# keonlee9420/Transformer-tacotron2

Measured on AMD Instinct MI355X. Metric: mel frames/sec (train step) at 1/2/4/8 GPUs; decode frames/sec b=32, higher is better.
Workload: dtype bf16; 1 GPU; train step (fwd+loss+bwd+Adam; one rank: no gradient exchange), LJSpeech-shape synthetic batch; global_batch=16, per_gpu_batch=16, seq_len=800, text_len=128, n_mels=80, params=52986691, parallelism=dp1, graph=True, optimizer=Adam at the end of each step

## Files before the change

transformer-tacotron2_amd/csrc/gemm.hip:

```cpp
#include "gemm_common.h"

using tt2g::Epilogue;
using tt2g::Operand;

#ifndef TT2_G10_AUTO
#define TT2_G10_AUTO 1
#endif
#ifndef TT2_G11_AUTO
#define TT2_G11_AUTO 1
#endif
#ifndef G11_MAX_K
#define G11_MAX_K 1024
#endif

extern "C" size_t tt2_gemm_workspace_size(const tt2_gemm_args* a) {
  if (a->splits <= 1) return 0;
  return (size_t)a->splits * a->m * (a->n + (a->a_ksum ? 1 : 0)) * sizeof(float);
}

static bool g7_lds_epi(int variant) { return variant != 13; }

#ifndef G8_SPLIT_TO_V7
#define G8_SPLIT_TO_V7 1
#endif
#ifndef G8_AUTO_TILES
#define G8_AUTO_TILES 64
#endif
#ifndef G8_SPLIT_MIN_K
#define G8_SPLIT_MIN_K 4096
#endif
namespace tt2g {
int gemm_plan(const tt2_gemm_args* a) {
  const int var = a->kernel_variant;
  const int64_t a_inner = a->trans_a ? a->m : a->k, b_inner = a->trans_b ? a->n : a->k;
  const bool half_in = a->dtype_in == TT2_BF16 || a->dtype_in == TT2_F16;
  const bool skinny = half_in && a->m <= 64 && !a->trans_a && !a->trans_b && a->k % 8 == 0 &&
                      a->a_conv_t == 0 && (a->splits <= 1 || a->main_only) && (var == 0 || var == 3);
  if (skinny && a->splits > 1 && (a->a_ln_gamma || a->kv_cache || a->pe_table || a->emit_mel ||
                                  a->k % (32 * a->splits) != 0))
    return tt2_set_error(TT2_E_INVALID, "tt2_gemm: skinny split-K slabs need k % (32 splits) == 0, no fusions"), -1;
  if ((a->a_ln_gamma || a->kv_cache) && !skinny)
    return tt2_set_error(TT2_E_INVALID, "tt2_gemm: a_ln / kv fusions need the skinny path (bf16, m <= 64, NT)"), -1;
  if (a->dtype_in == TT2_F16 && !skinny)
    return tt2_set_error(TT2_E_INVALID, "tt2_gemm: f16 operands only on the skinny decode path (m <= 64, NT)"), -1;
  if (a->a_ln_gamma && (a->dtype_in != TT2_BF16 || a->k != 512 || a->lda != a->k || a->m > 32 || !a->a_ln_branch ||
                        !a->a_ln_beta ||
                        !a->a_ln_out))
    return tt2_set_error(TT2_E_INVALID, "tt2_gemm: a_ln needs k == lda == 512, m <= 32, branch, beta and out"), -1;
  if (a->kv_cache && (!a->kv_t || a->dtype_out != a->dtype_in))
    return tt2_set_error(TT2_E_INVALID, "tt2_gemm: kv scatter needs kv_t and an output of the input dtype"), -1;
  if ((a->pe_table || a->emit_mel) && !skinny)
    return tt2_set_error(TT2_E_INVALID, "tt2_gemm: pe / emit epilogues need the skinny path (bf16, m <= 64, NT)"), -1;
  if (a->pe_table && (!a->pe_alpha || !a->pe_t))
    return tt2_set_error(TT2_E_INVALID, "tt2_gemm: pe epilogue needs pe_alpha and pe_t"), -1;
  if (a->emit_mel && (!a->emit_stop || !a->emit_prev || !a->emit_t || !a->emit_done || a->emit_nmels >= a->n ||
                      a->emit_nmels <= 0 || a->emit_tmax <= 0))
    return tt2_set_error(TT2_E_INVALID, "tt2_gemm: emit epilogue needs stop/prev/t/done and n > emit_nmels"), -1;
  if (skinny) return 3;
  const bool v2 = a->dtype_in == TT2_BF16 && var != 1 && a_inner % 8 == 0 && b_inner % 8 == 0;
  if (a->a_ksum && !(v2 && a->trans_a && a->a_conv_t == 0))
    return tt2_set_error(TT2_E_INVALID, "tt2_gemm: a_ksum needs bf16, trans_a, no conv A, the LDS-DMA kernel"), -1;
  if (!v2) return 1;
  auto conv_ok = [](int t, int c) { return t == 0 || (t >= 64 && c >= 64); };
  const bool v7ok = conv_ok(a->a_conv_t, a->a_conv_c) && conv_ok(a->b_conv_t, a->b_conv_c) &&
                    (int64_t)(a->trans_a ? a->k : a->m) * a->lda * 2 < (1LL << 31) &&
                    (int64_t)(a->trans_b ? a->k : a->n) * a->ldb * 2 < (1LL << 31);
  const bool v8ok = !a->trans_a && !a->a_ksum && a->b_conv_t == 0 && a->dtype_out == TT2_BF16 && a->n % 8 == 0 &&
                    !(a->splits > 1 && a->main_only) &&
                    (int64_t)a->m * a->lda * 2 < (1LL << 31) &&
                    (int64_t)(a->trans_b ? a->k : a->n) * a->ldb * 2 < (1LL << 31);
  const int64_t tiles7 = (int64_t)((a->m + 255) / 256) * ((a->n + 127) / 128);
  const bool split_v7 = G8_SPLIT_TO_V7 && a->splits > 1 && v7ok && a->k >= G8_SPLIT_MIN_K;
  if (v8ok && a->m >= 64 && (var == 15 || (var == 0 && tiles7 <= G8_AUTO_TILES && !split_v7))) return 15;
  const bool v10ok = v7ok && !a->trans_a && !a->trans_b && a->a_conv_t == 0 && !a->a_ksum &&
                     a->dtype_out == TT2_BF16 && a->splits <= 1 && a->n % 256 == 0 && a->k % 64 == 0 &&
                     !a->res && !a->gate && a->beta == 0.f && a->act != ACT_TANH &&
                     reinterpret_cast<uintptr_t>(a->c) % 16 == 0 && a->ldc % 8 == 0 &&
                     reinterpret_cast<uintptr_t>(a->bias) % 16 == 0;
  const int64_t cus = tt2_cu_count();
  const int64_t rounds7 = (tiles7 + cus - 1) / cus, rounds10 = ((a->m + 255) / 256 * (a->n / 256) + cus - 1) / cus;
  if (v10ok && (var == 16 || (var == 0 && TT2_G10_AUTO && 17 * rounds10 < 10 * rounds7))) return 16;
  const bool v11ok = v7ok && !a->trans_a && a->a_conv_t == 0 && a->b_conv_t == 0 && !a->a_ksum &&
                     a->dtype_out == TT2_BF16 && a->splits <= 1 && a->n % 128 == 0 && a->k % 64 == 0 &&
                     a->beta == 0.f && a->act != ACT_TANH && !a->col_stats && !a->bn_bwd &&
                     (a->trans_b ? !a->bias && !a->act && !a->drop_thr && !(a->res && a->gate)
                                 : !a->res && !a->gate) &&
                     reinterpret_cast<uintptr_t>(a->c) % 16 == 0 && a->ldc % 8 == 0 &&
                     reinterpret_cast<uintptr_t>(a->bias) % 16 == 0;
  if (v11ok && (var == 17 || (var == 0 && TT2_G11_AUTO && a->k <= G11_MAX_K && !a->trans_b))) return 17;
  if ((var == 13 || var == 14 || var == 0) && v7ok) return 13;
  return 2;
}
}

extern "C" int tt2_gemm_plan(const tt2_gemm_args* a) { return tt2g::gemm_plan(a); }

static bool epi_vec_ok(const tt2_gemm_args* a) {
  auto ok = [](const void* p, int64_t ld, int dt) {
    if (!p) return true;
    const int esz = dt == TT2_BF16 ? 2 : 4;
    return reinterpret_cast<uintptr_t>(p) % 16 == 0 && (ld * esz) % 16 == 0 && (8 * esz) % 16 == 0;
  };
  return a->dtype_out != TT2_F16 && a->res_dtype != TT2_F16 && a->gate_dtype != TT2_F16 &&
         ok(a->c, a->ldc, a->dtype_out) && ok(a->res, a->ldr, a->res_dtype) && ok(a->gate, a->ldg, a->gate_dtype) &&
         (reinterpret_cast<uintptr_t>(a->bias) % 16 == 0);
}

struct Route { int kernel, code, stats_rows; };

static int replan(const tt2_gemm_args* a, int variant) {
  tt2_gemm_args b = *a;
  b.kernel_variant = variant;
  return tt2g::gemm_plan(&b);
}

static Route gemm_route(const tt2_gemm_args* a, bool stats) {
  Route r{tt2g::gemm_plan(a), 0, 0};
  if (r.kernel < 0) return r;
  const bool vec = epi_vec_ok(a);
  if (r.kernel == 15 && !vec) r.kernel = replan(a, 13);
  if (stats) {
    auto al = [](const void* p, int64_t ld) { return reinterpret_cast<uintptr_t>(p) % 16 == 0 && (ld * 2) % 16 == 0; };
    bool ok = a->splits <= 1 && a->dtype_out == TT2_BF16 && al(a->c, a->ldc) && a->n % 8 == 0 &&
              (reinterpret_cast<uintptr_t>(a->col_stats) & 3) == 0;
    if (ok && r.kernel != 15) {
      ok = (r.kernel == 13 || replan(a, 14) == 13) && !a->trans_a && !a->trans_b &&
           g7_lds_epi(a->kernel_variant) && a->n % 128 == 0;
      if (ok) r.kernel = 13;
    }
    r.stats_rows = !ok ? 0 : r.kernel == 15 ? 64 : 256;
    return r;
  }
  if (r.kernel == 16 && (r.code = tt2g::g10_code(a, vec)) < 0) r.kernel = replan(a, 13);
  if (r.kernel == 17 && (r.code = tt2g::g11_code(a, vec)) < 0) r.kernel = replan(a, 13);
  return r;
}

extern "C" int32_t tt2_gemm_stats_rows(const tt2_gemm_args* a) { return gemm_route(a, true).stats_rows; }

int tt2g::gemm_prep(const tt2_gemm_args* a, Operand& A, Operand& B, Epilogue& ep) {
  const int esz = a->dtype_in == TT2_F32 ? 4 : 2;
  const int E = 16 / esz;
  auto misaligned = [&](const void* p, int64_t ld) {
    return (reinterpret_cast<uintptr_t>(p) % 16) != 0 || (ld * esz) % 16 != 0;
  };
  if (!a->a || !a->b || !a->c) return tt2_set_error(TT2_E_INVALID, "tt2_gemm: null operand");
  if (misaligned(a->a, a->lda) || misaligned(a->b, a->ldb))
    return tt2_set_error(TT2_E_INVALID, "tt2_gemm: operands must be 16-B aligned with 16-B multiple leading dims");
  if (a->a_conv_t > 0 && (a->trans_a || a->a_conv_c % E != 0 || a->lda != a->a_conv_c))
    return tt2_set_error(TT2_E_INVALID, "tt2_gemm: conv A needs K-contiguous A, lda == C, C % chunk == 0");
  if (a->b_conv_t > 0 && (!a->trans_b || a->b_conv_c % E != 0 || a->ldb != a->b_conv_c))
    return tt2_set_error(TT2_E_INVALID, "tt2_gemm: conv B needs N-contiguous B, ldb == C, C % chunk == 0");
  if (a->splits > 1 && (!a->workspace || a->ws_bytes < tt2_gemm_workspace_size(a)))
    return tt2_set_error(TT2_E_INVALID, "tt2_gemm: split-K workspace too small");

  A = Operand{a->a, a->lda, 0, 0, a->a_conv_t, a->a_conv_c, a->a_conv_pad};
  B = Operand{a->b, a->ldb, 0, 0, a->b_conv_t, a->b_conv_c, a->b_conv_pad};
  if (!a->trans_a) { A.outer_max = a->m; A.inner_max = a->k; } else { A.outer_max = a->k; A.inner_max = a->m; }
  if (!a->trans_b) { B.outer_max = a->n; B.inner_max = a->k; } else { B.outer_max = a->k; B.inner_max = a->n; }
  if (a->k <= 0) return tt2_set_error(TT2_E_INVALID, "tt2_gemm: k must be > 0");

  ep = Epilogue{};
  ep.c = a->c; ep.ldc = a->ldc; ep.c_dt = a->dtype_out;
  ep.bias = a->bias;
  ep.res = a->res; ep.ldr = a->ldr; ep.res_dt = a->res_dtype;
  ep.gate = a->gate; ep.ldg = a->ldg; ep.gate_dt = a->gate_dtype; ep.gate_scale = a->gate_scale;
  ep.alpha = a->alpha; ep.beta = a->beta; ep.act = a->act;
  ep.drop = drop_of(a);
  if (ep.drop.thr && !ep.drop.seed) return tt2_set_error(TT2_E_INVALID, "tt2_gemm: dropout without seed");
  ep.n_log = a->n;
  ep.ksum = a->a_ksum;
  ep.ksum_beta = a->a_ksum_beta;
  ep.main_only = a->main_only;
  ep.cstats = a->col_stats;
  if (const tt2_bn_args* bn = a->bn_bwd) {
    if (bn->dtype != TT2_DT_BF16 || bn->c != a->n || bn->m != a->m || !bn->y || !bn->mean || !bn->rstd ||
        !bn->gamma || !bn->beta || !bn->workspace || a->col_stats || (bn->drop_thr && !bn->drop_seed))
      return tt2_set_error(TT2_E_INVALID, "tt2_gemm: bn_bwd needs a bf16 BatchNorm of this GEMM's m x n, its "
                                          "y / mean / rstd / gamma / beta, a chunk-sums workspace, no col_stats");
    ep.bnb.y = reinterpret_cast<const bf16*>(bn->y);
    ep.bnb.mean = bn->mean; ep.bnb.rstd = bn->rstd; ep.bnb.gamma = bn->gamma; ep.bnb.beta = bn->beta;
    ep.bnb.part = reinterpret_cast<float*>(bn->workspace);
    ep.bnb.drop = drop_of(bn);
    ep.bnb.act = bn->act;
  }
  ep.vec = epi_vec_ok(a);
  return TT2_OK;
}

extern "C" int tt2_gemm(const tt2_gemm_args* a, hipStream_t stream) {
  ProbeDisarm disarm;
  if (a->m <= 0 || a->n <= 0) return TT2_OK;
  Operand A, B;
  Epilogue ep;
  if (const int rc = tt2g::gemm_prep(a, A, B, ep); rc != TT2_OK) return rc;
  float* ws = reinterpret_cast<float*>(a->workspace);
  const int sp = a->splits > 1 ? a->splits : 1;
  const bool stats = ep.cstats || ep.bnb.part;
  const Route r = gemm_route(a, stats);
  if (r.kernel < 0) return TT2_E_INVALID;
  if (stats) {
    if (!r.stats_rows)
      return tt2_set_error(TT2_E_INVALID, "tt2_gemm: col_stats / bn_bwd need the v8 path or v7's LDS-image path "
                                          "(bf16 C, 16-B aligned rows, no split-K; v7: NT and n % 128 == 0)");
    const int rp = r.stats_rows;
    if (a->bn_bwd && a->bn_bwd->ws_bytes < (size_t)((a->m + rp - 1) / rp) * 2 * a->n * sizeof(float))
      return tt2_set_error(TT2_E_INVALID, "tt2_gemm: bn_bwd workspace smaller than its chunk sums");
  }
  const bool a_kc = !a->trans_a, b_kc = !a->trans_b;
  const int m = a->m, n = a->n, k = a->k;
  switch (r.kernel) {
    case 3:
      return tt2_check_launch(tt2g::launch_skinny(a, ep, stream), "tt2_gemm(skinny)");
    case 16:
      return tt2_check_launch(tt2g::launch10(A, B, ep, m, n, k, r.code, stream), "tt2_gemm(v10)");
    case 17:
      return tt2_check_launch(tt2g::launch11(A, B, ep, m, n, k, b_kc, r.code, stream), "tt2_gemm(v11)");
    case 15:
      return tt2_check_launch(tt2g::launch8(b_kc, A, B, ep, m, n, k, stream), "tt2_gemm(v8)");
    case 13:
      return tt2_check_launch(tt2g::launch7(a_kc, b_kc, A, B, ep, m, n, k, sp, ws, stream,
                                            g7_lds_epi(a->kernel_variant)), "tt2_gemm(v7)");
    case 2:
      return tt2_check_launch(tt2g::launch2(a_kc, b_kc, A, B, ep, m, n, k, sp, ws, stream), "tt2_gemm");
    default:
      return tt2_check_launch(tt2g::launch1(a->dtype_in == TT2_BF16, a_kc, b_kc, A, B, ep, m, n, k, sp, ws, stream),
                              "tt2_gemm");
  }
}
```

transformer-tacotron2_amd/csrc/gemm_common.h:

```cpp
#pragma once
#include <hip/hip_ext.h>

#include <algorithm>
#include <cstdlib>

#include "tt2_common.h"
#include "tt2_capi.h"
#include "tt2_internal.h"

#ifdef TT2_PHASE
#define TT2_SPAN_W 32
#else
#define TT2_SPAN_W 2
#endif

namespace tt2g {

struct Operand {
  const void* p;
  int64_t ld;
  int outer_max, inner_max;
  int conv_t, conv_c, conv_pad;
};

struct Epilogue {
  void* c; int64_t ldc; int c_dt;
  const float* bias;
  const void* res; int64_t ldr; int res_dt;
  const void* gate; int64_t ldg; int gate_dt; float gate_scale;
  float alpha, beta;
  int act;
  DropDesc drop;
  int n_log;
  int vec;
  float* ksum; float ksum_beta;
  int main_only;
  float* cstats;
  struct {
    const bf16* y; const float* mean; const float* rstd; const float* gamma; const float* beta;
    float* part;
    DropDesc drop;
    int act;
  } bnb;
};

int probe_take(hipEvent_t& e0, hipEvent_t& e1, unsigned long long*& span, int groups);
void probe_chunk(int slot, int wgs);
void probe_disarm();

hipError_t launch1(bool bf16_in, bool a_kc, bool b_kc, const Operand& A, const Operand& B, const Epilogue& E, int M,
                   int N, int K, int splits, float* ws, hipStream_t s);
hipError_t launch2(bool a_kc, bool b_kc, const Operand& A, const Operand& B, const Epilogue& E, int M, int N, int K,
                   int splits, float* ws, hipStream_t s);
void launch_splitk_reduce(const float* ws, int splits, const Epilogue& E, int M, int N, hipStream_t s);
int splitk_blocks(int M, int N, const Epilogue& E);
hipError_t launch_skinny(const tt2_gemm_args* a, const Epilogue& E, hipStream_t s);
hipError_t launch7(bool a_kc, bool b_kc, const Operand& A, const Operand& B, const Epilogue& E, int M, int N, int K,
                   int splits, float* ws, hipStream_t s, bool lds_epi);
hipError_t launch8(bool b_kc, const Operand& A, const Operand& B, const Epilogue& E, int M, int N, int K,
                   hipStream_t s);
int g10_code(const tt2_gemm_args* a, bool vec);
hipError_t launch10(const Operand& A, const Operand& B, const Epilogue& E, int M, int N, int K, int code,
                    hipStream_t s);
int g11_code(const tt2_gemm_args* a, bool vec);
hipError_t launch11(const Operand& A, const Operand& B, const Epilogue& E, int M, int N, int K, bool b_kc, int code,
                    hipStream_t s);

int gemm_prep(const tt2_gemm_args* a, Operand& A, Operand& B, Epilogue& ep);
int gemm_plan(const tt2_gemm_args* a);

}

namespace {

struct OpDesc : tt2g::Operand {};
struct EpiParams : tt2g::Epilogue {};

constexpr int NT = 256;
constexpr int BM = 128, BN = 128;

TT2_DEV void span_begin(unsigned long long* span, int* done) {
  if (span && threadIdx.x == 0) {
    *done = 0;
    asm volatile("s_waitcnt lgkmcnt(0)" ::: "memory");
    span[TT2_SPAN_W * blockIdx.x] = wall_clock64();
#ifdef TT2_PHASE
    span[TT2_SPAN_W * blockIdx.x + 2] = __builtin_amdgcn_s_memtime();
#endif
  }
}
TT2_DEV void span_end(unsigned long long* span, int* done, int waves) {
  if (span) {
    asm volatile("s_waitcnt vmcnt(0)" ::: "memory");
    if ((threadIdx.x & 63) == 0 && atomicAdd(done, 1) == waves - 1) {
#ifdef TT2_PHASE
      span[TT2_SPAN_W * blockIdx.x + 31] = __builtin_amdgcn_s_memtime();
#endif
      span[TT2_SPAN_W * blockIdx.x + 1] = wall_clock64();
    }
  }
}

struct ProbeScope {
  hipEvent_t e0 = nullptr, e1 = nullptr;
  unsigned long long* span = nullptr;
  int slot = -1;
  ProbeScope(hipStream_t s, int groups) {
    if ((slot = tt2g::probe_take(e0, e1, span, groups)) < 0) return;
    hipStreamCaptureStatus cs = hipStreamCaptureStatusNone;
    if (hipStreamIsCapturing(s, &cs) == hipSuccess && cs == hipStreamCaptureStatusActive) e0 = e1 = nullptr;
    (void)hipGetLastError();
  }
  bool ext() const { return e0 != nullptr; }
  void chunk(int wgs) const { if (slot >= 0) tt2g::probe_chunk(slot, wgs); }
};

struct ProbeDisarm {
  ~ProbeDisarm() { tt2g::probe_disarm(); }
};

TT2_DEV float ld_any(const void* p, int64_t i, int dt) {
  if (dt == TT2_F16) return (float)reinterpret_cast<const f16*>(p)[i];
  return dt == TT2_BF16 ? (float)reinterpret_cast<const bf16*>(p)[i] : reinterpret_cast<const float*>(p)[i];
}
TT2_DEV void st_any(void* p, int64_t i, int dt, float v) {
  if (dt == TT2_F16) reinterpret_cast<f16*>(p)[i] = (f16)v;
  else if (dt == TT2_BF16) reinterpret_cast<bf16*>(p)[i] = (bf16)v;
  else reinterpret_cast<float*>(p)[i] = v;
}

TT2_DEV float epi_value(const EpiParams& e, uint32_t seed, int m, int n, float v) {
  v *= e.alpha;
  if (e.bias) v += e.bias[n];
  if (e.res) v += ld_any(e.res, (int64_t)m * e.ldr + n, e.res_dt);
  if (e.act == ACT_RELU) v = fmaxf(v, 0.f);
  else if (e.act == ACT_TANH) v = tanhf(v);
  if (e.gate) v = ld_any(e.gate, (int64_t)m * e.ldg + n, e.gate_dt) != 0.f ? v * e.gate_scale : 0.f;
  if (e.drop.thr) v = drop_apply(e.drop, seed, (uint32_t)((int64_t)m * e.n_log + n), v);
  if (e.beta != 0.f) v += e.beta * ld_any(e.c, (int64_t)m * e.ldc + n, e.c_dt);
  return v;
}

__device__ __attribute__((aligned(64))) uint4 g_zero_page[64];

typedef __attribute__((address_space(1))) void gvoid_t;
typedef __attribute__((address_space(3))) void lvoid_t;

TT2_DEV int mc_swz(int k) { return ((k & 3) << 1) ^ (((k >> 3) & 1) << 3); }

TT2_DEV const void* chunk_src(const OpDesc& d, int outer, int inner) {
  bool ok = (outer < d.outer_max) & (inner < d.inner_max);
  int64_t off = (int64_t)outer * d.ld + inner;
  if (d.conv_t > 0) {
    const int ts = outer % d.conv_t + inner / d.conv_c - d.conv_pad;
    ok = ok & (ts >= 0) & (ts < d.conv_t);
    off -= (int64_t)d.conv_pad * d.conv_c;
  }
  const void* p = reinterpret_cast<const bf16*>(d.p) + off;
  return ok ? p : (const void*)g_zero_page;
}

template <bool KC>
TT2_DEV void frag2(Frag8<bf16>& f, const char* tile, int r0, int kk, int lane) {
  if (KC) {
    const int row = r0 + (lane & 15);
    const int h = 4 * kk + (lane >> 4);
    f.v = *reinterpret_cast<const bf16x8*>(tile + row * 128 + ((h ^ (row & 7)) << 4));
  } else {
    const int g = lane >> 4, q = (lane >> 2) & 3, p = lane & 3;
    const int c = (r0 + 4 * p) >> 3;
    typedef __attribute__((address_space(3))) short4v lds_s4;
    const int k_lo = 32 * kk + 8 * g + q;
    const int k_hi = k_lo + 4;
    const char* a0 = tile + k_lo * 256 + ((c ^ mc_swz(k_lo)) << 4) + ((p & 1) << 3);
    const char* a1 = tile + k_hi * 256 + ((c ^ mc_swz(k_hi)) << 4) + ((p & 1) << 3);
    short4v lo = __builtin_amdgcn_ds_read_tr16_b64_v4i16((lds_s4*)(a0));
    short4v hi = __builtin_amdgcn_ds_read_tr16_b64_v4i16((lds_s4*)(a1));
    union { short s[8]; bf16x8 v; } u;
    u.s[0] = lo[0]; u.s[1] = lo[1]; u.s[2] = lo[2]; u.s[3] = lo[3];
    u.s[4] = hi[0]; u.s[5] = hi[1]; u.s[6] = hi[2]; u.s[7] = hi[3];
    f.v = u.v;
  }
}

TT2_DEV void ld8_any(const void* p, int64_t off, int dt, float (&o)[8]) {
  if (dt == TT2_BF16) {
    const bf16x8 x = *reinterpret_cast<const bf16x8*>(reinterpret_cast<const bf16*>(p) + off);
#pragma unroll
    for (int j = 0; j < 8; ++j) o[j] = (float)x[j];
  } else {
    const float* q = reinterpret_cast<const float*>(p) + off;
    const f32x4 a = *reinterpret_cast<const f32x4*>(q), b = *reinterpret_cast<const f32x4*>(q + 4);
#pragma unroll
    for (int j = 0; j < 4; ++j) { o[j] = a[j]; o[4 + j] = b[j]; }
  }
}

TT2_DEV void unpack_lds8(const void* p, float (&t)[8]) {
  const bf16x8 x = *reinterpret_cast<const bf16x8*>(p);
#pragma unroll
  for (int j = 0; j < 8; ++j) t[j] = (float)x[j];
}
TT2_DEV void epi_calc8(const EpiParams& E, uint32_t seed, int m, int n0, const float (&v)[8], bool pre_b,
                       float (&o)[8], const void* res_l = nullptr, const void* gate_l = nullptr) {
  const int64_t off = (int64_t)m * E.ldc + n0;
  float t[8];
#pragma unroll
  for (int j = 0; j < 8; ++j) o[j] = pre_b ? v[j] : v[j] * E.alpha;
  if (E.bias && !pre_b) {
    const f32x4 a = *reinterpret_cast<const f32x4*>(E.bias + n0), b = *reinterpret_cast<const f32x4*>(E.bias + n0 + 4);
#pragma unroll
    for (int j = 0; j < 4; ++j) { o[j] += a[j]; o[4 + j] += b[j]; }
  }
  if (E.res) {
    if (res_l) unpack_lds8(res_l, t);
    else ld8_any(E.res, (int64_t)m * E.ldr + n0, E.res_dt, t);
#pragma unroll
    for (int j = 0; j < 8; ++j) o[j] += t[j];
  }
// ... 124 lines not shown
```

transformer-tacotron2_amd/csrc/gemm_v7_impl.h:

```cpp
#pragma once
#include "gemm_v7.h"

namespace {

#ifndef G7_REG
#define G7_REG 0
#endif

template <int NI>
TT2_DEV void g7_put(const u32x4 (&r)[NI], char* lds, int lane, int lw) {
#pragma unroll
  for (int i = 0; i < NI; ++i) *reinterpret_cast<u32x4*>(lds + (lw * NI + i) * 1024 + lane * 16) = r[i];
}

constexpr int G7_MAXP = 8;
struct G7Fin {
  const float* part;
  float* dst[3];
  float gb;
  int nb, C;
};
struct G7Group {
  G7Prob p[G7_MAXP];
  int np, items;
  int ibase;
  G7Fin fin;
  int fin_only;
};
constexpr int G7_FIN_WAVES = 4;

template <int SM>
TT2_DEV void g7_store_c(const G7Prob& P, char* smem, int m0, int n0, int nkt) {
  bf16* C = reinterpret_cast<bf16*>(P.E.c);
  constexpr bool st = SM == 1, sb = SM == 2;
  const int c = threadIdx.x & 15;
  float k[8], s1[8], s2[8];
  if (st) bf16x8_unpack(*reinterpret_cast<const u32x4*>(smem + g7_img_row(nkt, 0) + (c << 4)), k);
#pragma unroll
  for (int j = 0; j < 8; ++j) s1[j] = s2[j] = 0.f;
  constexpr int NR = (256 * 16 + G7_NT - 1) / G7_NT;
  constexpr int YB = NR / 2;
  u32x4 yv[YB];
  float mu[8], rs[8], ga[8], be[8];
  uint32_t seed = 0;
  auto load_y = [&](int i0) {
#pragma unroll
    for (int i = 0; i < YB; ++i) {
      const int r = (threadIdx.x >> 4) + (G7_NT / 16) * (i0 + i), m = min(m0 + r, P.M - 1);
      yv[i] = r < 256 ? *reinterpret_cast<const u32x4*>(P.E.bnb.y + (int64_t)m * P.N + n0 + 8 * c)
                      : u32x4{0, 0, 0, 0};
    }
  };
  if constexpr (sb) {
    const int n = n0 + 8 * c;
    load_y(0);
#pragma unroll
    for (int j = 0; j < 8; ++j) {
      mu[j] = P.E.bnb.mean[n + j]; rs[j] = P.E.bnb.rstd[n + j];
      ga[j] = P.E.bnb.gamma[n + j]; be[j] = P.E.bnb.beta[n + j];
    }
    seed = P.E.bnb.drop.thr ? *P.E.bnb.drop.seed : 0u;
  }
#pragma unroll
  for (int i = 0; i < NR; ++i) {
    if constexpr (sb) {
      if (i == YB) load_y(YB);
    }
    const int id = threadIdx.x + G7_NT * i;
    if (id >= 256 * 16) break;
    const int r = id >> 4, m = m0 + r, n = n0 + 8 * c;
    if (m < P.M && n < P.N) {
      const u32x4 v = *reinterpret_cast<const u32x4*>(smem + g7_img_row(nkt, r) + ((c ^ (r & 15)) << 4));
      u32x4* dst = reinterpret_cast<u32x4*>(C + (int64_t)m * P.E.ldc + n);
      __builtin_nontemporal_store(v, dst);
      if constexpr (st) {
        float f[8];
        bf16x8_unpack(v, f);
#pragma unroll
        for (int j = 0; j < 8; ++j) {
          const float d = f[j] - k[j];
          s1[j] += d;
          s2[j] += d * d;
        }
      }
      if constexpr (sb) {
        float d[8], yf[8];
        bf16x8_unpack(v, d);
        bf16x8_unpack(yv[i % YB], yf);
        const DropDesc& dd = P.E.bnb.drop;
        const uint32_t bits = dd.thr ? drop_bits8(seed, dd.site, (uint32_t)((int64_t)m * P.N + n), dd.thr) : 0xFFu;
        const float sc = dd.thr ? dd.scale : 1.f;
#pragma unroll
        for (int j = 0; j < 8; ++j) {
          const float keep = (bits >> j) & 1u ? sc : 0.f;
          const float xh = (yf[j] - mu[j]) * rs[j];
          const float z = act_f(P.E.bnb.act, xh * ga[j] + be[j]);
          const float dp = d[j] * keep * act_grad_from_out(P.E.bnb.act, z);
          s1[j] += dp;
          s2[j] += dp * xh;
        }
      }
    }
  }
  if constexpr (!st && !sb) return;
  else {
#pragma unroll
  for (int j = 0; j < 8; ++j) {
    s1[j] += __shfl_xor(s1[j], 16);
    s2[j] += __shfl_xor(s2[j], 16);
    s1[j] += __shfl_xor(s1[j], 32);
    s2[j] += __shfl_xor(s2[j], 32);
  }
  float* red = reinterpret_cast<float*>(smem + ((nkt + 2) % 3) * G7_STAGE);
  const int lane = threadIdx.x & 63, wave = threadIdx.x >> 6;
  if (lane < 16) {
#pragma unroll
    for (int j = 0; j < 8; ++j) {
      red[(wave * 128 + 8 * c + j) * 2 + 0] = s1[j];
      red[(wave * 128 + 8 * c + j) * 2 + 1] = s2[j];
    }
  }
  __syncthreads();
  const int t = threadIdx.x;
  if (t < 128 && n0 + t < P.N) {
    float S1 = 0.f, S2 = 0.f;
    for (int w = 0; w < G7_NT / 64; ++w) {
      S1 += red[(w * 128 + t) * 2 + 0];
      S2 += red[(w * 128 + t) * 2 + 1];
    }
    const float kt = __uint_as_float((uint32_t)*reinterpret_cast<const uint16_t*>(smem + g7_img_row(nkt, 0) +
                                                                                  2 * t) << 16);
    if constexpr (st) {
      const float nr = (float)min(256, P.M - m0);
      float* out = P.E.cstats + (int64_t)(m0 / 256) * 2 * P.N + n0 + t;
      out[0] = kt + S1 / nr;
      out[P.N] = fmaxf(S2 - S1 * S1 / nr, 0.f);
    } else {
      float* out = P.E.bnb.part + (int64_t)(m0 / 256) * 2 * P.N + n0 + t;
      out[0] = S1;
      out[P.N] = S2;
    }
  }
  }
}

template <bool BIAS, bool RELU, bool DROP, int PX>
TT2_DEV void g7_epi_fast(const EpiParams& E, const f32x4 (&acc)[4][4], const f32x4 (&pbias)[2][2], char* smem,
                         int nkt, int m0, int n0, int wm, int wn, int lane, uint64_t dbits) {
  const int q = lane >> 4;
#pragma unroll
  for (int i = 0; i < 4; ++i) {
    const int r = wm * 64 + 16 * i + (lane & 15), m = m0 + r;
#pragma unroll
    for (int pr = 0; pr < 2; ++pr) {
      float v[8];
#pragma unroll
      for (int rr = 0; rr < 4; ++rr) {
// ... 330 lines not shown
__global__ __launch_bounds__(G7_NT, 1) void gemm7_kernel(G7Prob P) {
  __shared__ __attribute__((aligned(1024))) char smem[G7_SMEM];
  __shared__ int span_done;
  G7_RT(0)
  span_begin(P.span, &span_done);
  const int u = xcd_item(blockIdx.x, P.items);
  g7_item<AK, BKC, SM>(P, u % (P.items / P.splits), u / (P.items / P.splits), smem, P.span);
  span_end(P.span, &span_done, G7_NT / 64);
  G7_RT(1)
}

template <bool AK, bool BKC>
__global__ __launch_bounds__(G7_NT, 1) void gemm7g_kernel(G7Group G) {
  __shared__ __attribute__((aligned(1024))) char smem[G7_SMEM];
  __shared__ int span_done;
  span_begin(G.p[0].span, &span_done);
  const int u = xcd_item(G.ibase + blockIdx.x, G.items);
  int p = 0;
#pragma unroll
  for (int i = 1; i < G7_MAXP; ++i)
    if (i < G.np && u >= G.p[i].item0) p = i;
  const G7Prob& P = G.p[p];
  const int local = u - P.item0, nt = P.items / P.splits;
  g7_item<AK, BKC>(P, local % nt, local / nt, smem, G.p[0].span);
  span_end(G.p[0].span, &span_done, G7_NT / 64);
}

__global__ void gemm_splitk_reduce(const float* ws, int splits, EpiParams E, int M, int N) {
  splitk_reduce_body(ws, splits, E, M, N, blockIdx.x, gridDim.x);
}

__global__ void gemm_splitk_reduce_g(G7Group G) {
  if (G.fin_only || (int)blockIdx.y == G.np) {
    const G7Fin& f = G.fin;
    const int o = blockIdx.x * G7_FIN_WAVES + (threadIdx.x >> 6), lane = threadIdx.x & 63;
    if (o >= 3 * f.C) return;
    const int which = o / f.C, c = o - which * f.C;
    float* dst = f.dst[which];
    if (!dst) return;
    const float* src = f.part + (int64_t)which * f.C + c;
    const int64_t rs = 3 * (int64_t)f.C;
    float acc[4] = {0.f, 0.f, 0.f, 0.f};
    int r = lane;
    for (; r + 192 < f.nb; r += 256) {
#pragma unroll
      for (int u = 0; u < 4; ++u) acc[u] += src[(r + 64 * u) * rs];
    }
    for (; r < f.nb; r += 64) acc[0] += src[r * rs];
    const float v = wave_sum((acc[0] + acc[1]) + (acc[2] + acc[3]));
    if (lane == 0) dst[c] = f.gb != 0.f ? f.gb * dst[c] + v : v;
    return;
  }
  const G7Prob& P = G.p[blockIdx.y];
  if (P.splits > 1) splitk_reduce_body(P.ws, P.splits, P.E, P.M, P.N, blockIdx.x, gridDim.x);
}

G7Prob g7_prob(const OpDesc& A, const OpDesc& B, const EpiParams& E, int M, int N, int K, int splits,
                            float* ws) {
  G7Prob P{A, B, E, M, N, K, K, 1, (N + 127) / 128, 0, 0, ws, 0, 0, -1, nullptr};
  if (splits > 1) {
    P.k_split = ((K + splits - 1) / splits + 63) / 64 * 64;
    P.splits = (K + P.k_split - 1) / P.k_split;
  }
  P.items = ((M + 255) / 256) * P.ntn * P.splits;
  return P;
}

int g7_fast_code(const G7Prob& P, bool fwd) {
  const EpiParams& E = P.E;
  if (!P.lds_epi || E.beta != 0.f || E.act == ACT_TANH) return -1;
  if (P.pre_x) {
    const bool alone = !E.bias && E.act == ACT_NONE && !E.drop.thr && (P.pre_x == 1 ? !E.gate : !E.res);
    return alone ? 7 + P.pre_x : -1;
  }
  if (E.res || E.gate) return -1;
  if (E.bias && !fwd) return -1;
  return (E.bias ? 1 : 0) | (E.act == ACT_RELU ? 2 : 0) | (E.drop.thr ? 4 : 0);
}

template <bool AK, bool BKC>
hipError_t launch7_t(const OpDesc& A, const OpDesc& B, const EpiParams& E, int M, int N, int K, int splits, float* ws,
                   hipStream_t s, bool lds_epi) {
  G7Prob P = g7_prob(A, B, E, M, N, K, splits, ws);
  P.lds_epi = lds_epi && P.splits == 1 && E.c_dt == TT2_BF16 && E.vec && (N % 8) == 0;
  P.pre_x = !P.lds_epi ? 0 : (E.res && E.res_dt == TT2_BF16) ? 1 : (E.gate && E.gate_dt == TT2_BF16) ? 2 : 0;
  P.epi_fast = g7_fast_code(P, AK && BKC);
  ProbeScope ps(s, P.items);
  P.span = ps.span;
  const int sm = E.cstats ? 1 : E.bnb.part ? 2 : 0;
  auto go = [&](auto kern) {
    if (ps.ext()) hipExtLaunchKernelGGL(kern, dim3(P.items), dim3(G7_NT), 0, s, ps.e0, ps.e1, 0, P);
    else hipLaunchKernelGGL(kern, dim3(P.items), dim3(G7_NT), 0, s, P);
  };
  if constexpr (AK && BKC) {
    if (sm == 1) go(gemm7_kernel<AK, BKC, 1>);
    else if (sm == 2) go(gemm7_kernel<AK, BKC, 2>);
    else go(gemm7_kernel<AK, BKC, 0>);
  } else {
    go(gemm7_kernel<AK, BKC, 0>);
  }
  if (P.splits > 1 && !E.main_only)
    tt2g::launch_splitk_reduce(ws, P.splits, E, M, N, s);
  return hipGetLastError();
}

}

namespace tt2g {

void launch_splitk_reduce(const float* ws, int splits, const Epilogue& E, int M, int N, hipStream_t s) {
  hipLaunchKernelGGL(gemm_splitk_reduce, dim3(splitk_blocks(M, N, E)), dim3(256), 0, s, ws, splits, EpiParams{E}, M, N);
}

int splitk_blocks(int M, int N, const Epilogue& E) {
  const int64_t per = ((N & 7) == 0 && E.vec) ? 8 : ((N & 3) == 0 ? 4 : 1);
  const int64_t items = std::max<int64_t>(((int64_t)M * N + per - 1) / per, M);
  const int64_t nb = (items + 255) / 256;
  return (int)(nb < 4096 ? nb : 4096);
}

hipError_t launch7(bool a_kc, bool b_kc, const Operand& A_, const Operand& B_, const Epilogue& E_, int M, int N, int K,
                   int splits, float* ws, hipStream_t s, bool lds_epi) {
  const OpDesc A{A_}, B{B_};
  const EpiParams E{E_};
  if (a_kc && b_kc) return launch7_t<true, true>(A, B, E, M, N, K, splits, ws, s, lds_epi);
  if (a_kc && !b_kc) return launch7_t<true, false>(A, B, E, M, N, K, splits, ws, s, lds_epi);
  if (!a_kc && b_kc) return launch7_t<false, true>(A, B, E, M, N, K, splits, ws, s, lds_epi);
  return launch7_t<false, false>(A, B, E, M, N, K, splits, ws, s, lds_epi);
}

}

extern "C" int tt2_gemm_grouped_fin(const tt2_gemm_args* probs, int n, const tt2_ln_args* fin,
                                    hipStream_t stream) {
  return tt2_gemm_grouped_ex(probs, n, fin, 0, stream);
}

extern "C" int tt2_gemm_grouped_ex(const tt2_gemm_args* probs, int n, const tt2_ln_args* fin, int max_groups,
                                   hipStream_t stream) {
  ProbeDisarm disarm;
  if (n <= 0 && !fin) return TT2_OK;
  if ((n > 0 && !probs) || n > G7_MAXP) return tt2_set_error(TT2_E_INVALID, "tt2_gemm_grouped: 1..8 problems");
  G7Group G{};
  if (fin && fin->m > 0) {
    if (!fin->defer_finalize || !fin->workspace || fin->c <= 0)
      return tt2_set_error(TT2_E_INVALID, "tt2_gemm_grouped_fin: fin must be a deferred LayerNorm backward");
    G.fin.part = reinterpret_cast<const float*>(fin->workspace);
    G.fin.dst[0] = fin->dgamma; G.fin.dst[1] = fin->dbeta; G.fin.dst[2] = fin->dbias;
    G.fin.gb = fin->grad_beta;
    G.fin.C = fin->c;
    G.fin.nb = (int)(tt2_layernorm_bwd_workspace_size(fin) / (3 * sizeof(float) * fin->c));
  }
  int reduce_blocks = 0, ta = -1, tb = -1, main_only = 1;
  for (int i = 0; i < n; ++i) {
    const tt2_gemm_args* a = probs + i;
    if (a->m <= 0 || a->n <= 0) continue;
    OpDesc A, B;
    EpiParams ep;
    if (const int rc = tt2g::gemm_prep(a, A, B, ep); rc != TT2_OK) return rc;
    if (tt2g::gemm_plan(a) != 13)
      return tt2_set_error(TT2_E_INVALID, "tt2_gemm_grouped: every problem must take the v7 kernel (bf16, "
                                          "8-aligned inner dims, conv T, C >= 64, no decode fusions)");
    if (a->col_stats || a->bn_bwd) return tt2_set_error(TT2_E_INVALID, "tt2_gemm_grouped: no col_stats / bn_bwd");
    if (ta < 0) { ta = a->trans_a; tb = a->trans_b; }
    if (a->trans_a != ta || a->trans_b != tb)
      return tt2_set_error(TT2_E_INVALID, "tt2_gemm_grouped: problems must share trans_a / trans_b");
    G7Prob P = g7_prob(A, B, ep, a->m, a->n, a->k, a->splits > 1 ? a->splits : 1,
                       reinterpret_cast<float*>(a->workspace));
    P.item0 = G.items;
    G.items += P.items;
    G.p[G.np++] = P;
    main_only &= a->main_only;
    if (P.splits > 1) {
      reduce_blocks = std::max(reduce_blocks, tt2g::splitk_blocks(a->m, a->n, ep));
    }
  }
  const int fin_blocks = G.fin.nb ? (3 * G.fin.C + G7_FIN_WAVES - 1) / G7_FIN_WAVES : 0;
  if (G.np == 0) {
    G.fin_only = 1;
    if (fin_blocks) hipLaunchKernelGGL(gemm_splitk_reduce_g, dim3(fin_blocks, 1), dim3(256), 0, stream, G);
    return tt2_check_launch(hipGetLastError(), "tt2_gemm_grouped");
  }
  const int grid = max_groups > 0 ? std::min(G.items, std::max(8, max_groups / 8 * 8)) : G.items;
  ProbeScope ps(stream, G.items);
  ps.chunk(grid);
  for (G.ibase = 0; G.ibase < G.items; G.ibase += grid) {
    const dim3 g(std::min(grid, G.items - G.ibase));
    G.p[0].span = ps.span ? ps.span + (size_t)TT2_SPAN_W * G.ibase : nullptr;
    hipEvent_t ev0 = G.ibase == 0 ? ps.e0 : nullptr, ev1 = G.ibase + grid >= G.items ? ps.e1 : nullptr;
#define TT2_G7G(A_, B_)                                                                                    \
  if (ps.ext())                                                                                          \
    hipExtLaunchKernelGGL((gemm7g_kernel<A_, B_>), g, dim3(G7_NT), 0, stream, ev0, ev1, 0, G);            \
  else                                                                                                   \
    hipLaunchKernelGGL((gemm7g_kernel<A_, B_>), g, dim3(G7_NT), 0, stream, G);
    if (!ta && !tb) { TT2_G7G(true, true) }
    else if (!ta && tb) { TT2_G7G(true, false) }
    else if (ta && !tb) { TT2_G7G(false, true) }
    else { TT2_G7G(false, false) }
#undef TT2_G7G
  }
  G.ibase = 0;
  G.p[0].span = nullptr;
  if (main_only) reduce_blocks = 0;
  G.fin_only = reduce_blocks == 0 && fin_blocks > 0;
  if (G.fin_only)
    hipLaunchKernelGGL(gemm_splitk_reduce_g, dim3(fin_blocks, 1), dim3(256), 0, stream, G);
  else if (reduce_blocks > 0)
    hipLaunchKernelGGL(gemm_splitk_reduce_g, dim3(std::max(reduce_blocks, fin_blocks), G.np + (fin_blocks ? 1 : 0)),
                       dim3(256), 0, stream, G);
  return tt2_check_launch(hipGetLastError(), "tt2_gemm_grouped");
}

extern "C" int tt2_gemm_grouped(const tt2_gemm_args* probs, int n, hipStream_t stream) {
  return tt2_gemm_grouped_fin(probs, n, nullptr, stream);
}
```

Baseline: 1.975 million frames/s.

## Add warp-specialized 256x256 TN GEMM kernel for f32-output weight gradients

Adds a new v12 GEMM kernel with 256x256 tiles, 12 waves per block (8 compute, 4 producer waves issuing global-to-LDS loads into a 5-slot ring) and transposed LDS reads, for bf16 TN problems with f32 C. Grouped GEMM calls now route eligible problems (m,n multiples of 256, no split-K, plain epilogue) to it by default, and run the remaining problems on v7 afterwards. The aim is more data reuse per tile and loads that overlap compute on the large weight-gradient GEMMs. In exchange it adds a second launch per grouped call and uses one block per CU with large LDS, which can leave fewer tiles than CUs for some shapes.

Result: no change. 1.991 million frames/s (median of 6 runs) (+0.8%).

```diff
diff --git a/transformer-tacotron2_amd/csrc/gemm.hip b/transformer-tacotron2_amd/csrc/gemm.hip
--- a/transformer-tacotron2_amd/csrc/gemm.hip
+++ b/transformer-tacotron2_amd/csrc/gemm.hip
@@ -65,6 +65,11 @@
   const bool v7ok = conv_ok(a->a_conv_t, a->a_conv_c) && conv_ok(a->b_conv_t, a->b_conv_c) &&
                     (int64_t)(a->trans_a ? a->k : a->m) * a->lda * 2 < (1LL << 31) &&
                     (int64_t)(a->trans_b ? a->k : a->n) * a->ldb * 2 < (1LL << 31);
+  if (var == 18) {
+    if (v7ok && g12_shape_ok(a)) return 18;
+    return tt2_set_error(TT2_E_INVALID, "tt2_gemm: variant 18 needs a v7-eligible TN request with f32 C, m and n "
+                                        "multiples of 256, plain operands, no split-K"), -1;
+  }
   const bool v8ok = !a->trans_a && !a->a_ksum && a->b_conv_t == 0 && a->dtype_out == TT2_BF16 && a->n % 8 == 0 &&
                     !(a->splits > 1 && a->main_only) &&
                     (int64_t)a->m * a->lda * 2 < (1LL << 31) &&
@@ -212,6 +217,11 @@
   switch (r.kernel) {
     case 3:
       return tt2_check_launch(tt2g::launch_skinny(a, ep, stream), "tt2_gemm(skinny)");
+    case 18: {
+      const tt2g::GroupedProb gp{A, B, ep, m, n, k};
+      ProbeScope ps(stream, tt2g::g12_items(&gp, 1));
+      return tt2_check_launch(tt2g::launch12g(&gp, 1, 0, stream, ps.span, ps.e0, ps.e1), "tt2_gemm(v12)");
+    }
     case 16:
       return tt2_check_launch(tt2g::launch10(A, B, ep, m, n, k, r.code, stream), "tt2_gemm(v10)");
     case 17:
diff --git a/transformer-tacotron2_amd/csrc/gemm_common.h b/transformer-tacotron2_amd/csrc/gemm_common.h
--- a/transformer-tacotron2_amd/csrc/gemm_common.h
+++ b/transformer-tacotron2_amd/csrc/gemm_common.h
@@ -65,6 +65,11 @@
 int g11_code(const tt2_gemm_args* a, bool vec);
 hipError_t launch11(const Operand& A, const Operand& B, const Epilogue& E, int M, int N, int K, bool b_kc, int code,
                     hipStream_t s);
+struct GroupedProb { Operand A, B; Epilogue E; int M, N, K; };
+bool g12_shape_ok(const tt2_gemm_args* a);
+int g12_items(const GroupedProb* pr, int np);
+hipError_t launch12g(const GroupedProb* pr, int np, int max_groups, hipStream_t s, unsigned long long* span,
+                     hipEvent_t e0, hipEvent_t e1);
 
 int gemm_prep(const tt2_gemm_args* a, Operand& A, Operand& B, Epilogue& ep);
 int gemm_plan(const tt2_gemm_args* a);
diff --git a/transformer-tacotron2_amd/csrc/gemm_v12.hip b/transformer-tacotron2_amd/csrc/gemm_v12.hip
--- /dev/null
+++ b/transformer-tacotron2_amd/csrc/gemm_v12.hip
@@ -0,0 +1,267 @@
+#include "gemm_v7.h"
+
+namespace {
+
+constexpr int G12_NT = 768;
+constexpr int G12_SLOT = 256 * 128;
+constexpr int G12_SLOTS = 5;
+constexpr int G12_SMEM = G12_SLOTS * G12_SLOT;
+constexpr int G12_MAXP = 8;
+
+struct G12Prob {
+  OpDesc A, B;
+  EpiParams E;
+  int M, N, K, ntn, item0;
+};
+struct G12Group {
+  G12Prob p[G12_MAXP];
+  int np, items;
+  int ibase;
+  unsigned long long* span;
+};
+
+TT2_DEV uint32_t g12_lane_off(int lane) {
+  const int g = lane >> 4, q = (lane >> 2) & 3, p = lane & 3, k = 8 * g + q;
+  return (uint32_t)(k * 256 + (((p >> 1) ^ mc_swz(k)) << 4) + ((p & 1) << 3));
+}
+typedef __attribute__((address_space(3))) char lchar_t;
+TT2_DEV void g12_frag(Frag8<bf16>& fr, const lchar_t* smem, uint32_t off, int fx, int kk) {
+  typedef __attribute__((address_space(3))) short4v lds_s4;
+  const lchar_t* a0 = smem + (off ^ (uint32_t)fx) + 8192 * kk;
+  short4v lo = __builtin_amdgcn_ds_read_tr16_b64_v4i16((lds_s4*)(a0));
+  short4v hi = __builtin_amdgcn_ds_read_tr16_b64_v4i16((lds_s4*)(a0 + 1024));
+  union { short s[8]; bf16x8 v; } u;
+  u.s[0] = lo[0]; u.s[1] = lo[1]; u.s[2] = lo[2]; u.s[3] = lo[3];
+  u.s[4] = hi[0]; u.s[5] = hi[1]; u.s[6] = hi[2]; u.s[7] = hi[3];
+  fr.v = u.v;
+}
+
+typedef uint32_t g12_u32x2 __attribute__((ext_vector_type(2)));
+template <int OFF>
+TT2_DEV g12_u32x2 g12_tr_asm(uint32_t addr) {
+  g12_u32x2 r;
+  asm volatile("ds_read_b64_tr_b16 %0, %1 offset:%2" : "=v"(r) : "v"(addr), "n"(OFF));
+  return r;
+}
+
+TT2_DEV void g12_wait(int n) {
+  if (n >= 24) asm volatile("s_waitcnt vmcnt(24)" ::: "memory");
+  else if (n >= 16) asm volatile("s_waitcnt vmcnt(16)" ::: "memory");
+  else if (n >= 8) asm volatile("s_waitcnt vmcnt(8)" ::: "memory");
+  else asm volatile("s_waitcnt vmcnt(0)" ::: "memory");
+}
+
+__global__ __launch_bounds__(G12_NT, 1) void gemm12g_kernel(G12Group G) {
+  __shared__ __attribute__((aligned(1024))) char smem[G12_SMEM];
+  const int tid = threadIdx.x, lane = tid & 63, wave = __builtin_amdgcn_readfirstlane(tid >> 6);
+  unsigned long long* span = G.span;
+  if (span && tid == 0) span[TT2_SPAN_W * blockIdx.x] = wall_clock64();
+#ifdef TT2_PHASE
+  unsigned long long* srec = span ? span + TT2_SPAN_W * blockIdx.x : nullptr;
+  if (srec && tid == 0) srec[2] = __builtin_amdgcn_s_memtime();
+#endif
+  const int u = xcd_item(G.ibase + blockIdx.x, G.items);
+  int p = 0;
+#pragma unroll
+  for (int i = 1; i < G12_MAXP; ++i)
+    if (i < G.np && u >= G.p[i].item0) p = i;
+  const G12Prob& P = G.p[p];
+  const OpDesc& A = P.A;
+  const OpDesc& B = P.B;
+  const EpiParams& E = P.E;
+  const int tile = u - P.item0, ntn = P.ntn, K = P.K;
+  const int m0 = (tile / ntn) * 256, n0 = (tile % ntn) * 256;
+  const int nkt = (K + 63) / 64, nit = 2 * nkt;
+  if (wave >= 8) {
+    const int lw = wave - 8;
+    const bool tail = (K & 63) != 0;
+    G7Lane<8> la, lb;
+    g7_lane_init<false>(la, A, m0, 0, lane, lw);
+    g7_lane_init<false>(lb, B, n0, 0, lane, lw);
+    auto issue = [&](int it) {
+      char* dst = smem + (it % G12_SLOTS) * G12_SLOT;
+      const int t = it >> 1;
+      const bool tl = tail && t == nkt - 1;
+      if (it & 1) g7_issue<false>(B, lb, dst, 64 * t, K, lane, lw, tl, false);
+      else g7_issue<false>(A, la, dst, 64 * t, K, lane, lw, tl, false);
+    };
+    const bool do_ks = E.ksum && (tile % ntn) == 0;
+    f32x4 ksa[4];
+#pragma unroll
+    for (int ii = 0; ii < 4; ++ii) ksa[ii] = f32x4{0.f, 0.f, 0.f, 0.f};
+    Frag8<bf16> fones;
+#pragma unroll
+    for (int e = 0; e < 8; ++e) fones.v[e] = (bf16)1.f;
+    const uint32_t lk0 = (uint32_t)(uintptr_t)(const lchar_t*)smem +
+                         ((g12_lane_off(lane) + (lw >> 1) * 16384) ^ (uint32_t)((lw & 1) << 7));
+    const int pre = min(G12_SLOTS, nit);
+    for (int it = 0; it < pre; ++it) issue(it);
+    g12_wait(8 * (pre - 2));
+    __builtin_amdgcn_s_barrier();
+    for (int t = 0; t < nkt; ++t) {
+      if (t >= 1) {
+        if (2 * t + 3 < nit) issue(2 * t + 3);
+        if (2 * t + 4 < nit) issue(2 * t + 4);
+      }
+      if (do_ks) {
+        const uint32_t oa = ((2 * t) % G12_SLOTS) * G12_SLOT + lk0;
+        g12_u32x2 r[4][4];
+#pragma unroll
+        for (int ii = 0; ii < 4; ++ii) {
+          const uint32_t a = oa ^ (uint32_t)(ii << 5);
+          r[ii][0] = g12_tr_asm<0>(a);
+          r[ii][1] = g12_tr_asm<1024>(a);
+          r[ii][2] = g12_tr_asm<8192>(a);
+          r[ii][3] = g12_tr_asm<9216>(a);
+        }
+        asm volatile("s_waitcnt lgkmcnt(0)" ::: "memory");
+        __builtin_amdgcn_sched_barrier(0);
+#pragma unroll
+        for (int kk = 0; kk < 2; ++kk)
+#pragma unroll
+          for (int ii = 0; ii < 4; ++ii) {
+            union { g12_u32x2 h[2]; bf16x8 v; } u;
+            u.h[0] = r[ii][2 * kk];
+            u.h[1] = r[ii][2 * kk + 1];
+            Frag8<bf16> fa;
+            fa.v = u.v;
+            mma16(fones, fa, ksa[ii]);
+          }
+      }
+      if (t + 1 < nkt) {
+        const int last = min(nit - 1, max(G12_SLOTS - 1, 2 * t + 4));
+        g12_wait(8 * (last - (2 * t + 3)));
+      }
+      __builtin_amdgcn_s_barrier();
+    }
+    if (do_ks) {
+#pragma unroll
+      for (int ii = 0; ii < 4; ++ii) {
+        const float ks = ksa[ii][0];
+        const int m = m0 + 16 * (4 * lw + ii) + lane;
+        if (lane < 16) E.ksum[m] = E.ksum_beta != 0.f ? E.ksum_beta * E.ksum[m] + ks : ks;
+      }
+    }
+  } else {
+    const int wm = wave >> 2, wn = wave & 3, q = lane >> 4;
+    f32x4 acc[8][4];
+#pragma unroll
+    for (int i = 0; i < 8; ++i)
+#pragma unroll
+      for (int j = 0; j < 4; ++j) acc[i][j] = f32x4{0.f, 0.f, 0.f, 0.f};
+#if G7_PRIO
+    if (wave >= 4) __builtin_amdgcn_s_setprio(1);
+#endif
+    const lchar_t* sl = (const lchar_t*)smem;
+    const uint32_t la0 = g12_lane_off(lane) + wm * 16384;
+    const uint32_t lb0 = (g12_lane_off(lane) ^ (uint32_t)((wn & 1) << 7)) + (wn >> 1) * 16384;
+    __builtin_amdgcn_s_barrier();
+    for (int t = 0; t < nkt; ++t) {
+      G7_STAMP(t, 0)
+      uint32_t oa = ((2 * t) % G12_SLOTS) * G12_SLOT + la0, ob = ((2 * t + 1) % G12_SLOTS) * G12_SLOT + lb0;
+      asm volatile("" : "+v"(oa), "+v"(ob));
+      Frag8<bf16> fb[4], fa[2];
+#pragma unroll
+      for (int j = 0; j < 4; ++j) g12_frag(fb[j], sl, ob, j << 5, 0);
+      g12_frag(fa[0], sl, oa, 0, 0);
+#pragma unroll
+      for (int b = 0; b < 16; ++b) {
+        const int i = b & 7;
+        if (b + 1 < 16) g12_frag(fa[(b + 1) & 1], sl, oa, ((b + 1) & 7) << 5, (b + 1) >> 3);
+#pragma unroll
+        for (int j = 0; j < 4; ++j) {
+          mma16(fb[j], fa[b & 1], acc[i][j]);
+          if (b == 7) g12_frag(fb[j], sl, ob, j << 5, 1);
+        }
+        __builtin_amdgcn_sched_barrier(0);
+      }
+      G7_STAMP(t, 1)
+      asm volatile("s_waitcnt lgkmcnt(0)" ::: "memory");
+      __builtin_amdgcn_s_barrier();
+    }
+    G7_STAMP(nkt, 0)
+    float* C = reinterpret_cast<float*>(E.c);
+    const float alpha = E.alpha, beta = E.beta;
+#pragma unroll
+    for (int i = 0; i < 8; ++i) {
+      const int m = m0 + wm * 128 + 16 * i + (lane & 15);
+#pragma unroll
+      for (int pr = 0; pr < 2; ++pr) {
+        float v[8];
+#pragma unroll
+        for (int r = 0; r < 4; ++r) {
+          const auto sw = __builtin_amdgcn_permlane16_swap(__float_as_uint(acc[i][2 * pr][r]),
+                                                           __float_as_uint(acc[i][2 * pr + 1][r]), false, false);
+          v[r] = __uint_as_float(sw[0]);
+          v[4 + r] = __uint_as_float(sw[1]);
+        }
+        const int n = n0 + wn * 64 + 16 * (2 * pr + (q & 1)) + 8 * (q >> 1);
+        float* c = C + (int64_t)m * E.ldc + n;
+        float o[8];
+#pragma unroll
+        for (int j = 0; j < 8; ++j) o[j] = v[j] * alpha;
+        if (beta != 0.f) {
+          const f32x4 t0 = *reinterpret_cast<const f32x4*>(c), t1 = *reinterpret_cast<const f32x4*>(c + 4);
+#pragma unroll
+          for (int j = 0; j < 4; ++j) { o[j] += beta * t0[j]; o[4 + j] += beta * t1[j]; }
+        }
+        *reinterpret_cast<f32x4*>(c) = f32x4{o[0], o[1], o[2], o[3]};
+        *reinterpret_cast<f32x4*>(c + 4) = f32x4{o[4], o[5], o[6], o[7]};
+      }
+    }
+    G7_STAMP(nkt, 3)
+  }
+  if (span) {
+    asm volatile("s_waitcnt vmcnt(0)" ::: "memory");
+    __syncthreads();
+#ifdef TT2_PHASE
+    if (tid == 0) span[TT2_SPAN_W * blockIdx.x + 31] = __builtin_amdgcn_s_memtime();
+#endif
+    if (tid == 0) span[TT2_SPAN_W * blockIdx.x + 1] = wall_clock64();
+  }
+}
+
+}
+
+namespace tt2g {
+
+bool g12_shape_ok(const tt2_gemm_args* a) {
+  return a->dtype_in == TT2_BF16 && a->trans_a && a->trans_b && a->dtype_out == TT2_F32 && a->m % 256 == 0 &&
+         a->n % 256 == 0 && a->a_conv_t == 0 && a->b_conv_t == 0 && a->splits <= 1 && !a->col_stats && !a->bn_bwd &&
+         !a->bias && !a->res && !a->gate && a->act == ACT_NONE && !a->drop_thr &&
+         reinterpret_cast<uintptr_t>(a->c) % 16 == 0 && a->ldc % 4 == 0;
+}
+
+hipError_t launch12g(const GroupedProb* pr, int np, int max_groups, hipStream_t s, unsigned long long* span,
+                     hipEvent_t e0, hipEvent_t e1) {
+  if (np <= 0 || np > G12_MAXP) return hipErrorInvalidValue;
+  G12Group G{};
+  for (int i = 0; i < np; ++i) {
+    G12Prob& P = G.p[i];
+    P.A = OpDesc{pr[i].A};
+    P.B = OpDesc{pr[i].B};
+    P.E = EpiParams{pr[i].E};
+    P.M = pr[i].M; P.N = pr[i].N; P.K = pr[i].K;
+    P.ntn = P.N / 256;
+    P.item0 = G.items;
+    G.items += (P.M / 256) * P.ntn;
+  }
+  G.np = np;
+  const int grid = max_groups > 0 ? std::min(G.items, std::max(8, max_groups / 8 * 8)) : G.items;
+  for (G.ibase = 0; G.ibase < G.items; G.ibase += grid) {
+    const dim3 g(std::min(grid, G.items - G.ibase));
+    G.span = span ? span + (size_t)TT2_SPAN_W * G.ibase : nullptr;
+    hipEvent_t ev0 = G.ibase == 0 ? e0 : nullptr, ev1 = G.ibase + grid >= G.items ? e1 : nullptr;
+    if (ev0 || ev1) hipExtLaunchKernelGGL(gemm12g_kernel, g, dim3(G12_NT), 0, s, ev0, ev1, 0, G);
+    else hipLaunchKernelGGL(gemm12g_kernel, g, dim3(G12_NT), 0, s, G);
+  }
+  return hipGetLastError();
+}
+
+int g12_items(const GroupedProb* pr, int np) {
+  int items = 0;
+  for (int i = 0; i < np; ++i) items += (pr[i].M / 256) * (pr[i].N / 256);
+  return items;
+}
+
+}
diff --git a/transformer-tacotron2_amd/csrc/gemm_v7_impl.h b/transformer-tacotron2_amd/csrc/gemm_v7_impl.h
--- a/transformer-tacotron2_amd/csrc/gemm_v7_impl.h
+++ b/transformer-tacotron2_amd/csrc/gemm_v7_impl.h
@@ -3,6 +3,9 @@
 
 namespace {
 
+#ifndef TT2_G12_AUTO
+#define TT2_G12_AUTO 1
+#endif
 #ifndef G7_REG
 #define G7_REG 0
 #endif
@@ -639,19 +642,28 @@
     G.fin.nb = (int)(tt2_layernorm_bwd_workspace_size(fin) / (3 * sizeof(float) * fin->c));
   }
   int reduce_blocks = 0, ta = -1, tb = -1, main_only = 1;
+  tt2g::GroupedProb p12[G7_MAXP];
+  int n12 = 0;
   for (int i = 0; i < n; ++i) {
     const tt2_gemm_args* a = probs + i;
     if (a->m <= 0 || a->n <= 0) continue;
     OpDesc A, B;
     EpiParams ep;
     if (const int rc = tt2g::gemm_prep(a, A, B, ep); rc != TT2_OK) return rc;
-    if (tt2g::gemm_plan(a) != 13)
+    const int plan = tt2g::gemm_plan(a);
+    if (plan < 0) return TT2_E_INVALID;
+    if (plan != 13 && plan != 18)
       return tt2_set_error(TT2_E_INVALID, "tt2_gemm_grouped: every problem must take the v7 kernel (bf16, "
                                           "8-aligned inner dims, conv T, C >= 64, no decode fusions)");
     if (a->col_stats || a->bn_bwd) return tt2_set_error(TT2_E_INVALID, "tt2_gemm_grouped: no col_stats / bn_bwd");
     if (ta < 0) { ta = a->trans_a; tb = a->trans_b; }
     if (a->trans_a != ta || a->trans_b != tb)
       return tt2_set_error(TT2_E_INVALID, "tt2_gemm_grouped: problems must share trans_a / trans_b");
+    if (plan == 18 || (TT2_G12_AUTO && a->kernel_variant == 0 && tt2g::g12_shape_ok(a))) {
+      p12[n12++] = tt2g::GroupedProb{A, B, ep, a->m, a->n, a->k};
+      main_only &= a->main_only;
+      continue;
+    }
     G7Prob P = g7_prob(A, B, ep, a->m, a->n, a->k, a->splits > 1 ? a->splits : 1,
                        reinterpret_cast<float*>(a->workspace));
     P.item0 = G.items;
@@ -663,18 +675,23 @@
     }
   }
   const int fin_blocks = G.fin.nb ? (3 * G.fin.C + G7_FIN_WAVES - 1) / G7_FIN_WAVES : 0;
-  if (G.np == 0) {
+  if (G.np == 0 && n12 == 0) {
     G.fin_only = 1;
     if (fin_blocks) hipLaunchKernelGGL(gemm_splitk_reduce_g, dim3(fin_blocks, 1), dim3(256), 0, stream, G);
     return tt2_check_launch(hipGetLastError(), "tt2_gemm_grouped");
   }
-  const int grid = max_groups > 0 ? std::min(G.items, std::max(8, max_groups / 8 * 8)) : G.items;
-  ProbeScope ps(stream, G.items);
+  const int items12 = tt2g::g12_items(p12, n12), all = items12 + G.items;
+  const int grid = max_groups > 0 ? std::min(all, std::max(8, max_groups / 8 * 8)) : all;
+  ProbeScope ps(stream, all);
   ps.chunk(grid);
+  if (n12 > 0) {
+    const hipError_t e = tt2g::launch12g(p12, n12, max_groups, stream, ps.span, ps.e0, G.np == 0 ? ps.e1 : nullptr);
+    if (e != hipSuccess) return tt2_check_launch(e, "tt2_gemm_grouped(v12)");
+  }
   for (G.ibase = 0; G.ibase < G.items; G.ibase += grid) {
     const dim3 g(std::min(grid, G.items - G.ibase));
-    G.p[0].span = ps.span ? ps.span + (size_t)TT2_SPAN_W * G.ibase : nullptr;
-    hipEvent_t ev0 = G.ibase == 0 ? ps.e0 : nullptr, ev1 = G.ibase + grid >= G.items ? ps.e1 : nullptr;
+    G.p[0].span = ps.span ? ps.span + (size_t)TT2_SPAN_W * (items12 + G.ibase) : nullptr;
+    hipEvent_t ev0 = G.ibase == 0 && n12 == 0 ? ps.e0 : nullptr, ev1 = G.ibase + grid >= G.items ? ps.e1 : nullptr;
 #define TT2_G7G(A_, B_)                                                                                    \
   if (ps.ext())                                                                                          \
     hipExtLaunchKernelGGL((gemm7g_kernel<A_, B_>), g, dim3(G7_NT), 0, stream, ev0, ev1, 0, G);            \
@@ -687,7 +704,7 @@
 #undef TT2_G7G
   }
   G.ibase = 0;
-  G.p[0].span = nullptr;
+  if (G.np > 0) G.p[0].span = nullptr;
   if (main_only) reduce_blocks = 0;
   G.fin_only = reduce_blocks == 0 && fin_blocks > 0;
   if (G.fin_only)
```
